# hruffieux/atlasqtl

Measured on AMD Instinct MI355X. Metric: VB sweeps/sec, higher is better.
Workload: dtype f64; 1 GPU; atlasqtl VB sweep (S1-S22 incl. scheduled ELBO), n=1000 p=50000 q=10000, anneal=(1,2,10) on, horseshoe global-local, sweeps 6-93; n=1000, p=50000, q=10000, q_per_gpu=10000, parallelism=trait-sharded x1, env_overrides=

## Files before the change

### atlasqtl_amd/csrc/aq_core_sweep.h

```cpp
#pragma once
#include <hip/hip_runtime.h>
#include "aq_special.h"
#include "aq_plan_const.h"

typedef double aq_d4 __attribute__((ext_vector_type(4)));

struct AqCoreArgs {
  const double2 *XA;
  const double2 *XU;
  const double *G;
  const double *Gx;
  double *R;
  double *gam;
  double *mu;
  const double *Aarr;
  const double *Barr;
  const double *coef;
  const double *inv2s;
  const double *cst;
  const double *sig2b;
  double *sums;
  double *rowGB;
  double c;
  int p, q;
  int p_pad, q_pad, n_pad, nb, ntile;
  int dmode;
  int mode;
  int nseg;
  int stagger;
  int *done;
  int *errflag;
  int C;
  int xtouch;
  int xhelper;
  double *Pbuf;
  int *pflag;
  double *rnpart;
  const double *mis;
  const double *GK;
  const double *tau, *log_tau;
  const double *sig2_inv_p, *log_sig2_inv_p;
  long long *dbg;
  const double *theta;
  const double *zeta;
  double sqrt_c;
  int c_is_one;
  int mprio;
  int hprio;
};

__device__ __forceinline__ aq_d4 aq_mfma(double a, double b, aq_d4 c) {
  return __builtin_amdgcn_mfma_f64_16x16x4f64(a, b, c, 0, 0, 0);
}
__device__ __forceinline__ void aq_lds_barrier() { asm volatile("s_waitcnt lgkmcnt(0)\n\ts_barrier" ::: "memory"); }
__device__ __forceinline__ int aq_drow(int dmode, int reg, int g) { return (dmode ? 1 : 4) * reg + (dmode ? 4 : 1) * g; }
```

### atlasqtl_amd/csrc/aq_core_sweep_la.h

```cpp
#pragma once
#include <hip/hip_runtime.h>
#include "aq_core_sweep.h"
#include <type_traits>

typedef double aq_v2 __attribute__((ext_vector_type(2)));

__device__ __forceinline__ double aq_row16_sum(double v) {
  auto step = [&](auto ctrl) __attribute__((always_inline)) {
    constexpr int C = decltype(ctrl)::value;
    const int lo = __builtin_amdgcn_update_dpp(0, __double2loint(v), C, 0xf, 0xf, false);
    const int hi = __builtin_amdgcn_update_dpp(0, __double2hiint(v), C, 0xf, 0xf, false);
    v += __hiloint2double(hi, lo);
  };
  step(std::integral_constant<int, 0xB1>{});
  step(std::integral_constant<int, 0x4E>{});
  step(std::integral_constant<int, 0x124>{});
  step(std::integral_constant<int, 0x128>{});
  return v;
}

#ifndef AQ_GLDS_AUX
#define AQ_GLDS_AUX 2
#endif
__device__ __forceinline__ void aq_glds16(const void *gsrc_lane, void *lds_base) {
// ... 724 lines not shown
          double gxn[CXC ? RPG : 1];
          if constexpr (CXC) {
#pragma unroll
            for (int r = 0; r < RPG; r++) gxn[r] = LGx[(b + 1) % 3][(hg + NG * r) * 16 + j];
          }
          __builtin_amdgcn_sched_barrier(0);
          double s = sb + m1o * dj;
          double mu = rc_coef * s;
          double x = fma(-(s * s), rc_K, cA);
          double gm = aq_sigmoid_neg_fast(x);
          double dl = gm * mu - m1o;
          sb = s_nx - g_next * dl;
          if (j2 < 16) {
            Sown[j2 / NG] -= gl[j2 / NG] * dl;
            s_nx = __shfl(Sown[j2 / NG], (j2 % NG) * NTR + ht, 64);
            __builtin_amdgcn_sched_barrier(0);
          }
#pragma unroll
          for (int r = (j / NG); r < RPG; r++)
            if (!(j2 < 16 && r == j2 / NG)) Sown[r] -= gl[r] * dl;
          if constexpr (CXC) {
#pragma unroll
            for (int r = 0; r < RPG; r++) cxn[r] = (j == 0 ? 0.0 : cxn[r]) + gxn[r] * dl;
          }
          wgam[j * NTR] = gm;
          wmu[j * NTR] = mu;
          wdel[j * NTR] = dl;
          m1o = m1o_n; cA = cA_n; dj = d_n;
          if (j == 7) tl_mark(need, 6);
        }
        }
        signal(6, b - seg_b0 + 1);
      };
      if constexpr (NT3 > 0) {
        run(std::integral_constant<int, (NT3 > 0 ? NT3 : 1)>{}, std::integral_constant<int, 2>{},
            [&](int i) __attribute__((always_inline)) { if (i >= 1 && i <= nblk) chain_block(seg_b0 + i - 1); });
      } else {
        for (int b = seg_b0; b < seg_b1; b++) chain_block(b);
      }
    } else if constexpr (NT3 > 0) {
      run(std::integral_constant<int, (NT3 > 0 ? NT3 : 1)>{}, std::integral_constant<int, 2>{}, no_hook);
    }
    __syncthreads();
  } else if (helper) {
    if (a.hprio == 3) __builtin_amdgcn_s_setprio(3);
    else if (a.hprio == 2) __builtin_amdgcn_s_setprio(2);
    else if (a.hprio == 1) __builtin_amdgcn_s_setprio(1);
    const size_t tbase = (size_t)(tile0 + (ht >> 4)) * a.p_pad * 16 + (ht & 15);
    const double zk = a.zeta[ktrait];
    typedef __attribute__((address_space(3))) const double aq_lds_cdouble;
    aq_lds_cdouble *ptab = (aq_lds_cdouble *)(__attribute__((address_space(3))) double *)Lpt;
    const double inv_sqrt_c = 1.0 / a.sqrt_c;
    const double cst_k = MASK ? 0.0 : a.cst[ktrait];
    double th[RPG];
    auto theta_load = [&](int b) __attribute__((always_inline)) {
#pragma unroll
      for (int r = 0; r < RPG; r++) th[r] = a.theta[16 * b + hg + NG * r];
    };
    double pg[MASK ? 1 : RPG], pm[MASK ? 1 : RPG];
    auto gm_load = [&](int b) __attribute__((always_inline)) {
      if constexpr (!MASK) {
#pragma unroll
        for (int r = 0; r < RPG; r++) {
          const size_t off = tbase + (size_t)(16 * b + hg + NG * r) * 16;
          pg[r] = a.gam[off];
          pm[r] = a.mu[off];
        }
      }
    };
    const double tau_k = MASK ? a.tau[ktrait] : 1.0;
    const double sig2_inv_h = MASK ? *a.sig2_inv_p : 0.0;
    const double cstna_k = MASK ? -(a.log_tau[ktrait] + *a.log_sig2_inv_p) / 2 : 0.0;
    auto gk_block = [&](int b) __attribute__((always_inline)) { return a.GK + ((size_t)tile0 * a.nb + b) * AQ_GK_STRIDE; };
    auto gk_dma = [&](int b, int par) __attribute__((always_inline)) {
      const char *src = (const char *)gk_block(b) + lane * 16;
#pragma unroll
      for (int i = 0; i < AQ_GK_DIAG / 128; i++) aq_glds16(src + 1024 * i, &LGk2[par][128 * i]);
      src += AQ_GK_DIAG * 8;
#pragma unroll
      for (int i = 0; i < 32; i++) aq_glds16(src + 1024 * i, &LGxk[128 * i]);
    };
    double pl_g[MASK ? RPG : 1], pl_m[MASK ? RPG : 1], pl_xn[MASK ? RPG : 1];
    double sv_g[MASK ? RPG : 1], sv_m[MASK ? RPG : 1], sv_xn[MASK ? RPG : 1], sv_th[MASK ? RPG : 1];
    auto pre_load = [&](int b) __attribute__((always_inline)) {
      const double *gk = gk_block(b);
#pragma unroll
      for (int r = 0; r < RPG; r++) {
        const size_t off = tbase + (size_t)(16 * b + hg + NG * r) * 16;
        const int jj = hg + NG * r;
        pl_g[r] = a.gam[off];
        pl_m[r] = a.mu[off];
        pl_xn[r] = gk[(jj * (jj + 1) / 2 + jj) * 16 + ht];
      }
    };
    auto stage_dma = [&](int b, int par, int b_next) __attribute__((always_inline)) {
#pragma unroll
      for (int r = 0; r < RPG; r++) {
        asm volatile("" : "+v"(pl_g[r]), "+v"(pl_m[r]), "+v"(pl_xn[r]), "+v"(th[r]) : : "memory");
        sv_g[r] = pl_g[r]; sv_m[r] = pl_m[r]; sv_xn[r] = pl_xn[r]; sv_th[r] = th[r];
      }
      gk_dma(b, par);
      if (b_next < seg_b1) { pre_load(b_next); theta_load(b_next); }
    };
    auto stage = [&](int b, int par) __attribute__((always_inline)) {
      double st_G[4], st_Gx[4], st_xn[MASK ? RPG : 1];
      if constexpr (MASK) {
#pragma unroll
        for (int r = 0; r < RPG; r++) { Lm1[par][lane + 64 * r] = sv_g[r] * sv_m[r]; st_xn[r] = sv_xn[r]; }
      } else {
#pragma unroll
        for (int r = 0; r < RPG; r++) Lm1[par][lane + 64 * r] = pg[r] * pm[r];
#pragma unroll
        for (int r = 0; r < 4; r++) {
          st_G[r] = a.G[(size_t)b * 256 + lane + 64 * r];
          const int bx = CXC ? (b + 1 < a.nb ? b + 1 : b) : b;
          st_Gx[r] = a.Gx[(size_t)bx * 256 + lane + 64 * r];
        }
      }
      double ls2r[MASK ? RPG : 1];
      if constexpr (MASK) {
#pragma unroll
        for (int r = 0; r < RPG; r++) {
          const int e = lane + 64 * r;
          const double is2 = a.c * (st_xn[r] + sig2_inv_h) * tau_k;
          const double s2 = aq_recip_pos(is2);
          const double ls2 = -aq_log_pos(is2);
          const double cf = a.c * s2 * tau_k;
          Lcoef[par][e] = cf;
          LK[par][e] = cf * cf * (a.c * 0.5 * is2);
          Ls2[par][e] = s2;
          Lls2[par][e] = ls2;
          Lxn[par][e] = st_xn[r];
          ls2r[r] = ls2;
        }
      }
      auto emitA = [&](int r, double A) __attribute__((always_inline)) {
        const int j = 16 * b + hg + NG * r, e = lane + 64 * r;
        const bool valid = kvalid && j < a.p;
        if constexpr (MASK) {
          LA[par][e] = a.c * ((valid ? A : 0.0) - 0.5 * ls2r[r] + cstna_k);
        } else {
          LA[par][e] = a.c * ((valid ? A : 0.0) + cst_k);
        }
      };
      auto emitZ = [&](int r, double zb, double za) __attribute__((always_inline)) {
        const int j = 16 * b + hg + NG * r, e = lane + 64 * r;
        const bool valid = kvalid && j < a.p;
        LB[par][e] = valid ? zb : 0.0;
        Laa[par][e] = valid ? za : 0.0;
      };
      auto emit2 = [&](int r, double A, double zb, double za) __attribute__((always_inline)) {
        const int j = 16 * b + hg + NG * r, e = lane + 64 * r;
        const bool valid = kvalid && j < a.p;
        LB[par][e] = valid ? zb : 0.0;
        Laa[par][e] = valid ? za : 0.0;
        if constexpr (MASK) LA[par][e] = a.c * ((valid ? A : 0.0) - 0.5 * Lls2[par][e] + cstna_k);
        else LA[par][e] = a.c * ((valid ? A : 0.0) + cst_k);
      };
      double uu[RPG];
      bool inr = true;
#pragma unroll
      for (int r = 0; r < RPG; r++) {
        uu[r] = (MASK ? sv_th[r] : th[r]) + zk;
        inr = inr && fabs(uu[r]) < AQ_PT_R && fabs(a.sqrt_c * uu[r]) < AQ_PT_R;
      }
      {
        constexpr int NC = AQ_PT_DEG + 1, S = AQ_PT_NI, F = NC * S;
        auto locate = [&](double x, double *xloc) __attribute__((always_inline)) {
          const double t = fmin(fabs(x) * (1.0 / AQ_PT_W), AQ_PT_NI * (1.0 - 0x1p-53));
          const int i = (int)t;
          *xloc = fma(2.0, t - (double)i, -1.0);
          return ptab + i;
        };
        {
          double co[2][NC], xl[2];
          auto fetch = [&](int r, auto setc) __attribute__((always_inline)) {
            constexpr int set = decltype(setc)::value;
            aq_lds_cdouble *pp = locate(uu[r], &xl[set]);
#pragma unroll
            for (int k = 0; k < NC; k++) co[set][k] = pp[k * S];
          };
          fetch(0, std::integral_constant<int, 0>{});
          aq_static_for<RPG>([&](auto rc) __attribute__((always_inline)) {
            constexpr int r = decltype(rc)::value, set = r & 1;
            if constexpr (r + 1 < RPG) fetch(r + 1, std::integral_constant<int, (r + 1) & 1>{});
            __builtin_amdgcn_sched_barrier(0);
            double pa = co[set][NC - 1];
#pragma unroll
            for (int k = NC - 2; k >= 0; k--) pa = fma(pa, xl[set], co[set][k]);
            emitA(r, uu[r] < 0.0 ? -pa : pa);
            __builtin_amdgcn_sched_barrier(0);
          });
        }
        {
          double co[2][2 * NC], xl[2];
          auto fetch = [&](int r, auto setc) __attribute__((always_inline)) {
            constexpr int set = decltype(setc)::value;
            aq_lds_cdouble *pp = locate(a.sqrt_c * uu[r], &xl[set]);
#pragma unroll
            for (int k = 0; k < NC; k++) {
              co[set][k] = pp[F + k * S];
              co[set][NC + k] = pp[2 * F + k * S];
            }
          };
          fetch(0, std::integral_constant<int, 0>{});
          aq_static_for<RPG>([&](auto rc) __attribute__((always_inline)) {
            constexpr int r = decltype(rc)::value, set = r & 1;
            if constexpr (r + 1 < RPG) fetch(r + 1, std::integral_constant<int, (r + 1) & 1>{});
            __builtin_amdgcn_sched_barrier(0);
            double pb = co[set][NC - 1], pd = co[set][2 * NC - 1];
#pragma unroll
            for (int k = NC - 2; k >= 0; k--) {
              pb = fma(pb, xl[set], co[set][k]);
              pd = fma(pd, xl[set], co[set][NC + k]);
            }
            const double d = uu[r] < 0.0 ? -pd : pd;
            emitZ(r, pb * inv_sqrt_c, uu[r] - 0.5 * inv_sqrt_c * (pb + d));
            __builtin_amdgcn_sched_barrier(0);
          });
        }
      }
      if (__builtin_expect(!__all(inr), 0)) {
#pragma unroll 1
        for (int r = 0; r < RPG; r++) {
          double ur = uu[0];
#pragma unroll
          for (int k = 1; k < RPG; k++) ur = (r == k) ? uu[k] : ur;
          double A, bM, dM, dummy;
          aq_probit_tab_eval<1>(ur, ptab, &A, &dummy, &dummy);
          aq_probit_tab_eval<2>(a.sqrt_c * ur, ptab, &dummy, &bM, &dM);
          emit2(r, A, bM * inv_sqrt_c, ur - 0.5 * inv_sqrt_c * (bM + dM));
        }
      }
      if constexpr (MASK) {
#ifdef AQ_DIAG_TIME
        const long long t_dma = __builtin_readcyclecounter();
#endif
        asm volatile("s_waitcnt vmcnt(0)" ::: "memory");
#ifdef AQ_DIAG_TIME
        dg_wait += __builtin_readcyclecounter() - t_dma;
#endif
      } else {
#pragma unroll
        for (int r = 0; r < 4; r++) {
          const int e = lane + 64 * r;
          LG[par][(e >> 4) * 32 + (e & 15)] = st_G[r];
          LGx[CXC ? (b + 1) % 3 : par][e] = st_Gx[r];
        }
      }
    };
    double cs0 = 0.0, cs1 = 0.0, cs2 = 0.0, cs3 = 0.0, cs5 = 0.0;
    auto finalize = [&](int b, int par) __attribute__((always_inline)) {
#pragma unroll
      for (int r = 0; r < RPG; r++) {
        const int e = lane + 64 * r, hj = hg + NG * r;
        const double gm = Lgam[par][e], mu = Lmu[par][e];
        const size_t off = tbase + (size_t)(16 * b + hj) * 16;
        if (lead) {
          a.gam[off] = gm;
          a.mu[off] = mu;
        }
        const int j = 16 * b + hj;
        double gb = 0.0;
        if (kvalid && j < a.p) {
          const double be = gm * mu;
          gb = Laa[par][e] + gm * LB[par][e];
          cs0 += gm;
          cs3 += gb;
          if constexpr (MASK) {
            const double s2 = Ls2[par][e];
            const double m2 = (mu * mu + s2) * gm;
            const double xn = Lxn[par][e];
            cs1 += m2;
            cs2 += xn * (m2 - be * be);
            cs5 += gm * Lls2[par][e];
          } else {
            cs1 += (mu * mu + sig2b_k) * gm;
            cs2 += be * be;
          }
        }
        gb = aq_row16_sum(gb);
        if ((ht & 15) == 0 && lead) a.rowGB[(size_t)(tile0 + (ht >> 4)) * a.p_pad + j] = gb;
      }
    };
    auto exchange = [&](int b) __attribute__((always_inline)) {
      const int par = b & 1, kdone = b - seg_b0 + 1;
      if constexpr (WIDE) tl_mark(kdone, 0);
#pragma unroll
      for (int m = 0; m < NWM; m++) wait_ge(m, kdone);
      if constexpr (NT3 > 0) wait_ge(11, kdone);
      if constexpr (WIDE) tl_mark(kdone, 1);
      double own[RPG];
#pragma unroll
      for (int r = 0; r < RPG; r++) {
        const int e = lane + 64 * r;
        double sv = Sp[par][0][e];
#pragma unroll
        for (int ww = 1; ww < NPS; ww++) sv += Sp[par][ww][e];
        own[r] = sv;
      }
      if constexpr (WIDE) split_exchange_wide(b, own, [] {});
      else split_exchange(b, own, [] {});
#pragma unroll
      for (int r = 0; r < RPG; r++) Stot[par][lane + 64 * r] = own[r];
      signal(14, kdone);
    };
    if (a.mode == 1) {
      for (int b = seg_b0; b < seg_b1; b++) {
        const int k = b - seg_b0, par = b & 1;
        if (k >= 2) {
#pragma unroll
          for (int m = 0; m < NWM; m++) wait_ge(m, k + 1);
          if (NT3 > 0) wait_ge(11, k + 1);
        }
#pragma unroll
        for (int r = 0; r < RPG; r++) {
          const int e = lane + 64 * r, hj = hg + NG * r;
          const size_t off = tbase + (size_t)(16 * b + hj) * 16;
          double gm = a.gam[off], mu = a.mu[off];
          double be = gm * mu;
          Ldel[par][e] = be;
          if (kvalid && (16 * b + hj) < a.p) {
            const double m2 = (mu * mu + sig2b_k) * gm;
            cs0 += gm;
            cs1 += m2;
            if constexpr (MASK) cs2 += gk_block(b)[(hj * (hj + 1) / 2 + hj) * 16 + ht] * (m2 - be * be);
            else cs2 += be * be;
          }
        }
        signal(6, k + 1);
      }
    } else {
      int xt[8] = {0, 0, 0, 0, 0, 0, 0, 0};
      const long long xt_blk = (long long)NTT * C * 2048;
      const int xt_nsl = (int)((xt_blk + 8191) / 8192);
      const int xt_wg = (int)(gridDim.x < 256 ? gridDim.x : 256) / 8 > 0 ? (int)(gridDim.x < 256 ? gridDim.x : 256) / 8 : 1;
      auto x_touch = [&](int bA, int bU) __attribute__((always_inline)) {
        asm volatile("s_waitcnt vmcnt(0)" : "+v"(xt[0]), "+v"(xt[1]), "+v"(xt[2]), "+v"(xt[3]), "+v"(xt[4]), "+v"(xt[5]), "+v"(xt[6]), "+v"(xt[7]));
        const char *pa = (const char *)a.XA + (long long)bA * xt_blk + lane * 128, *pu = (const char *)a.XU + (long long)bU * xt_blk + lane * 128;
#pragma unroll
        for (int k = 0; k < 4; k++) {
          const int sl = (int)((blockIdx.x >> 3) % xt_wg) + k * xt_wg;
          if (sl < xt_nsl && (long long)sl * 8192 + lane * 128 < xt_blk) {
            asm volatile("global_load_dword %0, %1, off" : "=v"(xt[2 * k]) : "v"(pa + (long long)sl * 8192));
            asm volatile("global_load_dword %0, %1, off" : "=v"(xt[2 * k + 1]) : "v"(pu + (long long)sl * 8192));
          }
        }
      };
      theta_load(seg_b0);
      gm_load(seg_b0);
      if constexpr (MASK) { pre_load(seg_b0); stage_dma(seg_b0, seg_b0 & 1, seg_b0 + 1); }
      stage(seg_b0, seg_b0 & 1);
      signal(7, 1);
      if constexpr (!SEG && TT == 1) { if (C > 1 && a.xhelper) exchange(seg_b0); }
      if constexpr (!MASK) { if (seg_b0 + 1 < seg_b1) { theta_load(seg_b0 + 1); gm_load(seg_b0 + 1); } }
      for (int b = seg_b0; b < seg_b1; b++) {
        const int par = b & 1;
        if constexpr (MASK) {
          if (b + 1 < seg_b1) { wait_ge(13, b - seg_b0 + 1); stage_dma(b + 1, par ^ 1, b + 2); }
        }
        if (b > seg_b0) {
          wait_ge(6, b - seg_b0);
          if constexpr (!MASK && !CXC) {
            double dlp[16];
#pragma unroll
            for (int i = 0; i < 16; i++) dlp[i] = Ldel[par ^ 1][i * NTR + ht];
#pragma unroll
            for (int r = 0; r < RPG; r++) {
              double cx = 0.0;
              const double *gx = &LGx[par][(hg + NG * r) * 16];
#pragma unroll
              for (int i = 0; i < 16; i++) cx += gx[i] * dlp[i];
              Lcx[lane + 64 * r] = cx;
            }
            signal(12, b - seg_b0 + 1);
          }
          finalize(b - 1, par ^ 1);
        }
        if (b + 1 < seg_b1) {
          stage(b + 1, par ^ 1);
          signal(7, b - seg_b0 + 2);
          if constexpr (!SEG && TT == 1) { if (C > 1 && a.xhelper) exchange(b + 1); }
          if (a.xtouch && b + 2 < seg_b1) x_touch(b + 2, b);
          if constexpr (!MASK) { if (b + 2 < seg_b1) { theta_load(b + 2); gm_load(b + 2); } }
        }
      }
      asm volatile("s_waitcnt vmcnt(0)" : "+v"(xt[0]), "+v"(xt[1]), "+v"(xt[2]), "+v"(xt[3]), "+v"(xt[4]), "+v"(xt[5]), "+v"(xt[6]), "+v"(xt[7]));
      wait_ge(6, nblk);
      finalize(seg_b1 - 1, (seg_b1 - 1) & 1);
    }
    Lred[0][lane] = cs0; Lred[1][lane] = cs1; Lred[2][lane] = cs2; Lred[3][lane] = cs3; Lred[5][lane] = cs5;
    __syncthreads();
  } else {
    if (mw < 3) run(std::integral_constant<int, NT>{}, std::integral_constant<int, 0>{}, no_hook);
    else run(std::integral_constant<int, NT2>{}, std::integral_constant<int, 1>{}, no_hook);
    __syncthreads();
  }
#ifdef AQ_DIAG_TIME
  if (lane == 0 && a.dbg) {
    a.dbg[((size_t)blockIdx.x * 8 + w) * 3] = dg_wait;
    a.dbg[((size_t)blockIdx.x * 8 + w) * 3 + 1] = dg_wait_b;
    a.dbg[((size_t)blockIdx.x * 8 + w) * 3 + 2] = __builtin_readcyclecounter() - dg_t0;
  }
#endif
  if (tid < NTR) {
    int k2 = tile0 * 16 + tid;
    double r2 = 0.0;
    for (int s = 0; s < NPS * 4; s++) r2 += Lrn[s][tid];
    double *sm = a.sums + (size_t)seg * (MASK ? 6 : 5) * a.q_pad;
    if (C > 1) a.rnpart[(size_t)part * a.q_pad + k2] = r2;
    else sm[(size_t)4 * a.q_pad + k2] = r2;
    for (int v = 0; v < 6 && lead; v++) {
      if (v == 4 || (v == 5 && !MASK)) continue;
      double acc2 = 0.0;
      for (int jj = 0; jj < NG; jj++) acc2 += Lred[v][jj * NTR + tid];
      sm[(size_t)v * a.q_pad + k2] = acc2;
    }
  }
  if (SEG) {
    asm volatile("s_waitcnt vmcnt(0)" ::: "memory");
    __syncthreads();
    if (tid == 0) {
      __builtin_amdgcn_fence(__ATOMIC_RELEASE, "agent");
      asm volatile("s_waitcnt vmcnt(0)" ::: "memory");
      __hip_atomic_store(&a.done[wg], seg + 1, __ATOMIC_RELAXED, __HIP_MEMORY_SCOPE_AGENT);
    }
  }
}
```

### atlasqtl_amd/csrc/aq_plan.h

```cpp
#pragma once
#include <algorithm>
#include <cstdio>
#include <cstdlib>
#include <functional>
#include <string>

#include "../../include/atlasqtl_hip.h"
#include "aq_plan_const.h"

struct AqPlanInput {
  int n = 0, p = 0, q = 0;
  bool has_missing = false;
  int max_missing = 0;
  int max_short_list = 0;
  int ncu = 256;
  long long total_bytes = -1;
  const char *mem_error = nullptr;
};

struct AqPlan {
  bool use_la = false;
  bool use_mis = false;
  bool use_tw = false;
  bool la_mask = false;
  bool la_wide = false;
  int NT = 0;
  int NT2 = 0;
  int NT3x = -1;
  int TT = 1;
  int laC = 1;
  int misC = 1;
  int chain = 0;
  int stagger = 0;
  int la_xhelper = 0;
  int la_xtouch = 1;
  int la_hprio = 0;
  int la_mprio = 1;
  int NE = 0;
  int WPT = 1;
  int tw_ns = 4;
  int Mmax = 0, NR = 0;
  int p_pad = 0, q_pad = 0, n_pad = 0, nb = 0, ntile = 0;
  int ncu = 256;
};

using AqEnv = std::function<const char *(const char *)>;

enum AqHook { AQ_H_NCU, AQ_H_KERNEL, AQ_H_LA_C, AQ_H_GK_MAX_GB, AQ_H_MIS_C, AQ_H_TW_WPT, AQ_H_TT, AQ_H_NT3, AQ_H_LA_NOSPLIT,
              AQ_H_LA_XHELPER, AQ_H_XTOUCH, AQ_H_MPRIO, AQ_H_HPRIO, AQ_H_STAGGER, AQ_H_CHAIN, AQ_H_COUNT };
static const char *const aq_hook_names[AQ_H_COUNT] = {"AQ_NCU", "AQ_KERNEL", "AQ_LA_C", "AQ_GK_MAX_GB", "AQ_MIS_C", "AQ_TW_WPT", "AQ_TT", "AQ_NT3",
                                                      "AQ_LA_NOSPLIT", "AQ_LA_XHELPER", "AQ_XTOUCH", "AQ_MPRIO", "AQ_HPRIO", "AQ_STAGGER", "AQ_CHAIN"};
struct AqOpt { bool set = false, seen = false; int v = 0; double d = 0.0; };
struct AqHooks {
  const AqEnv &env;
  AqOpt opt[AQ_H_COUNT];
  const AqOpt &operator[](AqHook h) {
    AqOpt &o = opt[h];
    if (!o.seen) {
      o.seen = true;
      if (const char *v = env ? env(aq_hook_names[h]) : nullptr) { o.set = true; o.v = atoi(v); o.d = atof(v); }
    }
    return o;
  }
};

static inline int aq_plan_fail(std::string *err, int code, const std::string &msg) {
  if (err) *err = msg;
  return code;
}
static inline int aq_round16(int x) { return (x + 15) / 16 * 16; }

static inline int aq_plan_gk_budget(const AqPlanInput &in, AqHooks &h, bool wide, bool *la_mask_ok, std::string *err) {
  const size_t ntile_ = (size_t)(in.q + 15) / 16, nb_ = (size_t)(in.p + 15) / 16;
  const size_t gk_b = ntile_ * nb_ * AQ_GK_STRIDE * sizeof(double);
  const size_t rest_b = 2 * ntile_ * nb_ * 256 * sizeof(double) + 3 * (size_t)(in.n + 64) * nb_ * 16 * sizeof(double) * 2 +
                        3 * ntile_ * (size_t)(in.n + 64) * 16 * sizeof(double);
  const bool mem_known = in.total_bytes >= 0;
  if (wide && !mem_known) return aq_plan_fail(err, AQ_ERR_DEVICE, std::string("hipMemGetInfo: ") + (in.mem_error ? in.mem_error : "failed"));
  if (!mem_known || (!wide && (double)(gk_b + rest_b) * 1.05 > 0.9 * (double)in.total_bytes)) *la_mask_ok = false;
  const AqOpt &e = h[AQ_H_GK_MAX_GB];
  if (e.set && (double)gk_b > e.d * 1e9) *la_mask_ok = false;
  if (wide && !*la_mask_ok) {
    char msg[256];
    snprintf(msg, sizeof msg, "Y with missing values at n = %d: the per-trait Gram blocks need %.1f GB of device memory, which does not "
             "fit; shard the traits (fewer traits per device)", in.n, (double)gk_b / 1e9);
    return aq_plan_fail(err, AQ_ERR_UNSUPPORTED, msg);
  }
  return AQ_OK;
}

static inline int aq_plan_kernel(const AqPlanInput &in, AqHooks &h, AqPlan *pl, bool *wide_out, std::string *err) {
  const AqOpt &ek = h[AQ_H_KERNEL];
  const bool n_la_ok = in.n <= 8 * 16 * 105;
  const AqOpt &ecw = h[AQ_H_LA_C];
  const bool wide = in.n > 10240 || (ecw.set && ecw.v >= 9);
  if (wide && ecw.set && (ecw.v > AQ_LA_CMAX || (in.n > 10240 && ecw.v < 9)))
    return aq_plan_fail(err, AQ_ERR_ARG, "AQ_LA_C: the wide sample split takes 9 ... " + std::to_string(AQ_LA_CMAX) + " parts");
  if (wide && ek.set && ek.v >= 2) return aq_plan_fail(err, AQ_ERR_UNSUPPORTED, "AQ_KERNEL: only the look-ahead kernel serves n > 10240");
  bool la_mask_ok = in.has_missing && n_la_ok && in.max_missing <= AQ_MIS_MMAX && !(ek.set && ek.v >= 2);
  if (wide) la_mask_ok = in.has_missing;
  if (la_mask_ok) {
    const int rc = aq_plan_gk_budget(in, h, wide, &la_mask_ok, err);
    if (rc != AQ_OK) return rc;
  }
// ... 125 lines not shown
    if (tiles >= (1 << 30)) continue;
    const double rounds = (double)(((long long)pl->ntile * C + pl->ncu - 1) / pl->ncu);
    const double cost = rounds * std::max(0.213 * (NT + NT2) + 1.0, 4.5 + 0.2 * (C - 2));
    if (cost < best - 1e-9) { best = cost; pl->laC = C; pl->NT = NT; pl->NT2 = NT2; pl->NT3x = N3x; pl->n_pad = 16 * tiles * C; }
  }
  return best;
}

static inline double aq_plan_la_wide(AqPlan *pl, const AqOpt &ec, int ntiles) {
  auto helper_us = [](int C) { return 8.5 + 0.14 * (C - 12); };
  double best = 1e300;
  pl->la_wide = true;
  const int cf = ec.set ? ec.v : 0;
  for (int C = 9; C <= AQ_LA_CMAX && C <= pl->ncu; C++) {
    if (cf >= 9 && C != cf) continue;
    const int NT = ((ntiles + C - 1) / C + 5) / 6;
    if (NT > 18) continue;
    const double rounds = (double)(((long long)pl->ntile * C + pl->ncu - 1) / pl->ncu);
    const double cost = rounds * std::max(0.213 * 2 * NT + 1.0, helper_us(C));
    if (cost < best - 1e-9) { best = cost; pl->laC = C; pl->NT = NT; pl->NT2 = NT; pl->NT3x = -1; pl->n_pad = 16 * 6 * NT * C; }
  }
  return best;
}

static inline int aq_plan_la(const AqPlanInput &in, AqHooks &h, bool wide, AqPlan *pl, std::string *err) {
  const int ntiles = (in.n + 15) / 16;
  const bool split = !(in.n <= 1056 && !h[AQ_H_LA_C].set);
  pl->TT = (4LL * pl->ntile >= 7LL * pl->ncu) ? 2 : 1;
  const AqOpt &ett = h[AQ_H_TT];
  if (ett.set) pl->TT = ett.v == 2 ? 2 : 1;
  if (pl->la_mask) pl->TT = 1;
  if (split) pl->TT = 1;
  if (pl->TT == 2) {
    pl->q_pad = (in.q + 31) / 32 * 32;
    pl->ntile = pl->q_pad / 16;
  }
  const AqOpt &e3 = h[AQ_H_NT3];
  if (!split) {
    const int rc = aq_plan_la_unsplit(h, pl, e3, ntiles, err);
    if (rc != AQ_OK) return rc;
  } else {
    const AqOpt &ec = h[AQ_H_LA_C];
    const double best = wide ? aq_plan_la_wide(pl, ec, ntiles) : aq_plan_la_medium(pl, e3, ec, ntiles);
    if (best >= 1e300) return aq_plan_fail(err, AQ_ERR_UNSUPPORTED, "no look-ahead geometry for this n");
    pl->la_xhelper = wide ? 1 : 0;
  }
  if (h[AQ_H_LA_XHELPER].set) pl->la_xhelper = h[AQ_H_LA_XHELPER].v != 0;
  if (h[AQ_H_XTOUCH].set) pl->la_xtouch = h[AQ_H_XTOUCH].v != 0;
  if (pl->la_mask && pl->laC <= 1) pl->la_hprio = 1;
  if (pl->TT == 2 && pl->NT >= 8 && (pl->NT3x == 9 || (pl->NT3x < 0 && pl->NT2 == pl->NT - 1))) pl->la_hprio = 1;
  if (h[AQ_H_MPRIO].set) pl->la_mprio = h[AQ_H_MPRIO].v != 0;
  const AqOpt &ehp = h[AQ_H_HPRIO];
  if (ehp.set) pl->la_hprio = ehp.v >= 0 && ehp.v <= 3 ? ehp.v : 0;
  if (pl->TT == 2) pl->stagger = (pl->NT + 2) / 3;
  const AqOpt &est = h[AQ_H_STAGGER];
  if (est.set) pl->stagger = est.v >= 0 ? est.v : 0;
  pl->chain = aq_plan_chain(h, false, pl->ntile / pl->TT, pl->nb, pl->ncu, pl->laC > 1);
  if (pl->la_wide) pl->Mmax = pl->la_mask ? aq_round16(in.max_short_list) : 0;
  else if (pl->la_mask) pl->Mmax = aq_round16(in.max_missing);
  if ((pl->la_wide || pl->la_mask) && pl->Mmax < 16) pl->Mmax = 16;
  if (pl->la_mask) pl->NR = pl->n_pad + 8;
  return AQ_OK;
}

static inline int aq_plan_wide_budget(const AqPlanInput &in, const AqPlan &pl, std::string *err) {
  const double xb = 2.0 * (double)pl.nb * (pl.n_pad / 16) * 128 * sizeof(double);
  const double rb = (pl.la_mask ? 2.0 : 1.0) * (double)pl.ntile * pl.n_pad * 16 * sizeof(double);
  const double gb = pl.la_mask ? (double)pl.ntile * pl.nb * AQ_GK_STRIDE * sizeof(double) + (double)pl.nb * (pl.n_pad + 8) * 16 * sizeof(double) +
                                     (double)pl.ntile * 16 * pl.Mmax * sizeof(int)
                               : 0.0;
  if (in.total_bytes < 0) return aq_plan_fail(err, AQ_ERR_DEVICE, "hipMemGetInfo failed");
  if ((xb + rb + gb) * 1.05 > 0.9 * (double)in.total_bytes) {
    char msg[256];
    snprintf(msg, sizeof msg, "n = %d, p = %d, q = %d: the wide sample split needs %.1f GB of device memory, more than the device holds; "
             "shard the traits (fewer traits per device)", in.n, in.p, in.q, (xb + rb + gb) * 1.05 / 1e9);
    return aq_plan_fail(err, AQ_ERR_UNSUPPORTED, msg);
  }
  return AQ_OK;
}

static inline int aq_make_plan(const AqPlanInput &in, const AqEnv &env, AqPlan *out, std::string *err) {
  if (in.n > AQ_N_MAX)
    return aq_plan_fail(err, AQ_ERR_UNSUPPORTED, "n = " + std::to_string(in.n) + " exceeds the largest supported sample count, n <= " +
                                                     std::to_string(AQ_N_MAX) + " (AQ_N_MAX, the wide sample split)");
  AqHooks h{env, {}};
  AqPlan pl;
  pl.p_pad = aq_round16(in.p);
  pl.q_pad = aq_round16(in.q);
  pl.nb = pl.p_pad / 16;
  pl.ntile = pl.q_pad / 16;
  pl.ncu = in.ncu;
  if (h[AQ_H_NCU].set && h[AQ_H_NCU].v > 0) pl.ncu = h[AQ_H_NCU].v;
  bool wide = false;
  int rc = aq_plan_kernel(in, h, &pl, &wide, err);
  if (rc != AQ_OK) return rc;
  if (pl.use_mis) aq_plan_mis(in, h, &pl);
  else if (pl.use_tw) aq_plan_tw(in, h, &pl);
  else rc = aq_plan_la(in, h, wide, &pl, err);
  if (rc == AQ_OK && pl.la_wide) rc = aq_plan_wide_budget(in, pl, err);
  if (rc != AQ_OK) return rc;
  *out = pl;
  return AQ_OK;
}

static inline int aq_core_kernel_id(const AqPlan &pl) { return pl.use_mis ? 3 : pl.use_tw ? 2 : 0; }
static inline void aq_plan_to_status(const AqPlan &pl, aq_vb_status *st) {
// ... 11 lines not shown
```

### atlasqtl_amd/csrc/aq_vb_create.hip

```cpp
#include <hip/hip_runtime.h>

#include <algorithm>
#include <cmath>
#include <cstdlib>
#include <cstring>
#include <memory>
#include <string>
#include <vector>

#include "aq_vb.h"
#include "aq_setup_kernels.h"

static int aq_upload_padded(double *dst, const double *src, size_t n, size_t n_pad) {
  AQ_HIP(hipMemset(dst, 0, n_pad * sizeof(double)));
  AQ_HIP(hipMemcpy(dst, src, n * sizeof(double), hipMemcpyHostToDevice));
  return AQ_OK;
}

static AqEnv aq_env_recorder(std::string *found) {
  return [found](const char *name) {
    const char *v = getenv(name);
    if (v) *found += (found->empty() ? "" : " ") + std::string(name) + "=" + v;
    return v;
  };
}

extern "C" int64_t aq_vb_reduce_len(int32_t p) { return (int64_t)((p + 15) / 16) * 16 + AQ_RED_EXTRA; }

static std::vector<double> aq_ladder(const double anneal[3]) {
  double k_m = 1.0 / anneal[1];
  int m = (int)std::llround(anneal[2]);
  std::vector<double> l(m);
  int type = (int)std::llround(anneal[0]);
  if (type == 1) {
    double delta = std::pow(k_m, 1.0 / (1 - m)) - 1;
    for (int i = 0; i < m; i++) l[i] = std::pow(1 + delta, 1.0 - (double)(m - i));
  } else if (type == 2) {
    double delta = (1 / k_m - 1) / (m - 1);
    for (int i = 0; i < m; i++) l[i] = 1.0 / (1 + delta * ((double)(m - i) - 1));
  } else {
    double delta = (1 - k_m) / (m - 1);
    for (int i = 0; i < m; i++) l[i] = k_m + delta * (double)i;
  }
  return l;
}


static void aq_fill_args(aq_vb *s) {
  AqCoreArgs &a = s->core_args;
  a.XA = s->XA.get(); a.XU = s->XU.get(); a.G = s->G.get(); a.Gx = s->Gx.get(); a.R = s->R.get(); a.gam = s->gam.get(); a.mu = s->mu.get();
  a.theta = s->theta.get(); a.zeta = s->zeta.get();
  a.Aarr = s->Aarr.get(); a.Barr = s->Barr.get(); a.coef = s->coef.get(); a.inv2s = s->inv2s.get(); a.cst = s->cst.get(); a.sig2b = s->sig2b.get();
  a.sums = s->sums.get(); a.rowGB = s->rowGB.get();
  a.p = s->p; a.q = s->q; a.p_pad = s->p_pad; a.q_pad = s->q_pad; a.n_pad = s->n_pad; a.nb = s->nb; a.ntile = s->ntile;
  a.dmode = s->dmode;
  a.done = s->done.get(); a.errflag = s->errflag.get(); a.stagger = s->stagger;
  a.C = s->laC; a.xhelper = s->la_xhelper; a.Pbuf = s->Pbuf.get(); a.pflag = s->pflag.get(); a.rnpart = s->rnpart.get();
  a.xtouch = s->la_xtouch;
  a.hprio = s->la_hprio;
  a.mprio = s->la_mprio;
  a.mis = s->mis.get(); a.GK = s->GK.get(); a.tau = s->tau.get(); a.log_tau = s->log_tau.get();
  a.sig2_inv_p = &s->sc.get()->sig2_inv; a.log_sig2_inv_p = &s->sc.get()->log_sig2_inv;

  AqMisArgs &m = s->mis_args;
  m.XA = s->XA.get(); m.XU = s->XU.get(); m.G = s->G.get(); m.XR = s->XR.get(); m.R = s->R.get(); m.mis = s->mis.get(); m.gam = s->gam.get(); m.mu = s->mu.get();
  m.Aarr = s->Aarr.get(); m.Barr = s->Barr.get(); m.tau = s->tau.get(); m.log_tau = s->log_tau.get(); m.sig2b = s->sig2b.get(); m.sc = s->sc.get();
  m.midx = s->midx.get(); m.mcnt4 = s->mcnt4.get(); m.sums = s->sums.get(); m.rowGB = s->rowGB.get();
  m.p = s->p; m.q = s->q; m.p_pad = s->p_pad; m.q_pad = s->q_pad; m.n_pad = s->n_pad; m.nb = s->nb; m.ntile = s->ntile;
  m.dmode = s->dmode; m.NR = s->NR; m.Mmax = s->Mmax;
  m.C = s->misC; m.Pbuf = s->Pbuf.get(); m.pflag = s->pflag.get(); m.errflag = s->errflag.get(); m.rnpart = s->rnpart.get();
  m.done = s->done.get();

  AqTwArgs &t = s->tw_args;
  t.X = s->Xcm.get(); t.R = s->R.get(); t.mis = s->mis.get(); t.XN = s->XN.get(); t.gam = s->gam.get(); t.mu = s->mu.get(); t.Aarr = s->Aarr.get(); t.Barr = s->Barr.get();
  t.tau = s->tau.get(); t.log_tau = s->log_tau.get(); t.sig2b = s->sig2b.get(); t.sc = s->sc.get(); t.sums = s->sums.get(); t.rowGB = s->rowGB.get();
  t.n = s->n; t.p = s->p; t.q = s->q; t.n_pad = s->n_pad; t.p_pad = s->p_pad; t.q_pad = s->q_pad; t.ntile = s->ntile;
  t.complete = s->has_missing ? 0 : 1;
  t.ns = s->tw_ns;

  AqPrepass &v = s->pre_args;
  v.theta = s->theta.get(); v.zeta = s->zeta.get(); v.gam = s->gam.get(); v.Aarr = s->Aarr.get(); v.Barr = s->Barr.get(); v.rowA = s->rowA.get();
  v.colApart = s->colApart.get(); v.Hpart = s->Hpart.get(); v.p = s->p; v.q = s->q; v.p_pad = s->p_pad; v.q_pad = s->q_pad;
  v.rows_per_chunk = s->rows_per_chunk;
  v.write_AB = s->fused ? 0 : 1;

  AqQvec &qv = s->qv;
  qv.eta_h = s->eta_h.get(); qv.kappa_h = s->kappa_h.get(); qv.n0 = s->n0.get(); qv.nobs = s->nobs.get();
  qv.zeta = s->zeta.get(); qv.tau = s->tau.get(); qv.sig2b = s->sig2b.get(); qv.log_tau = s->log_tau.get(); qv.eta_vb = s->eta_vb.get();
  qv.kappa_vb = s->kappa_vb.get(); qv.coef = s->coef.get(); qv.inv2s = s->inv2s.get(); qv.cst = s->cst.get(); qv.sums = s->sums.get();
  qv.colApart = s->colApart.get(); qv.nchunk = s->fused ? 0 : s->nHchunk;
  qv.q = s->q; qv.q_pad = s->q_pad; qv.n = s->n; qv.nu_h = s->nu; qv.rho_h = s->rho;
  qv.na = s->has_missing ? 1 : 0;

  AqPvec &pv = s->pv;
  pv.theta = s->theta.get(); pv.sig2_theta = s->sig2_theta.get(); pv.L = s->L.get(); pv.lam2_inv = s->lam2_inv.get(); pv.Q = s->Q.get();
  pv.rsZ = s->red; pv.part = s->ppart.get(); pv.p = s->p; pv.p_pad = s->p_pad; pv.shr = s->shr; pv.m0 = s->m0;
  pv.A2_inv = s->A2_inv; pv.df = (double)s->df;
}

extern "C" int aq_vb_create(const aq_vb_problem *pr, aq_vb_handle *out) {
  if (!pr || !out) return aq_fail(AQ_ERR_ARG, "aq_vb_create: NULL argument");
  *out = nullptr;
  if (pr->n < 2 || pr->p < 1 || pr->q < 1) return aq_fail(AQ_ERR_ARG, "aq_vb_create: n >= 2, p >= 1, q >= 1 required");
  if (pr->q_total < pr->q) return aq_fail(AQ_ERR_ARG, "aq_vb_create: q_total < q");
  if (!pr->X || !pr->Y || !pr->eta || !pr->kappa || !pr->n0 || (!pr->init_generate && (!pr->gam_vb || !pr->mu_beta_vb)) || !pr->sig2_beta_vb ||
      !pr->sig2_theta_vb || !pr->tau_vb || !pr->theta_vb || !pr->zeta_vb)
    return aq_fail(AQ_ERR_ARG, "aq_vb_create: NULL data pointer");
  if (!(pr->tol > 0)) return aq_fail(AQ_ERR_ARG, "tol must be positive");
  if (pr->maxit < 1) return aq_fail(AQ_ERR_ARG, "maxit must be natural.");
  if (pr->has_anneal) {
    int type = (int)std::llround(pr->anneal[0]);
    if (type < 1 || type > 3)
// ... 275 lines not shown
```

Before: 29.36 sweeps/s.

## Specialize helper loop for c==1 and all-valid blocks with scalar base addressing

Splits the helper wave's block loop into template-specialized variants. One handles c==1 (annealing finished), reusing the polynomial table lookup and dropping the sqrt_c scaling. Another skips per-row validity checks for interior blocks. Loads and stores of gamma, mu, G, Gx, theta and rowGB now use wave-uniform scalar bases (readfirstlane) with 32-bit lane offsets, and rowGB is written with one selected store instead of a per-row conditional store. This cuts VALU address arithmetic and branching on the helper path, at the cost of code size from three instantiated loop bodies.

```diff
diff --git a/atlasqtl_amd/csrc/aq_core_sweep.h b/atlasqtl_amd/csrc/aq_core_sweep.h
--- a/atlasqtl_amd/csrc/aq_core_sweep.h
+++ b/atlasqtl_amd/csrc/aq_core_sweep.h
@@ -47,6 +47,7 @@
   int c_is_one;
   int mprio;
   int hprio;
+  int hfast;
 };
 
 __device__ __forceinline__ aq_d4 aq_mfma(double a, double b, aq_d4 c) {
diff --git a/atlasqtl_amd/csrc/aq_core_sweep_la.h b/atlasqtl_amd/csrc/aq_core_sweep_la.h
--- a/atlasqtl_amd/csrc/aq_core_sweep_la.h
+++ b/atlasqtl_amd/csrc/aq_core_sweep_la.h
@@ -800,19 +800,33 @@
     aq_lds_cdouble *ptab = (aq_lds_cdouble *)(__attribute__((address_space(3))) double *)Lpt;
     const double inv_sqrt_c = 1.0 / a.sqrt_c;
     const double cst_k = MASK ? 0.0 : a.cst[ktrait];
+    auto ubase = [&](const void *p0, long long byteoff) __attribute__((always_inline)) {
+      const unsigned long long v = (unsigned long long)((const char *)p0 + byteoff);
+      const unsigned lo = __builtin_amdgcn_readfirstlane((unsigned)v), hi = __builtin_amdgcn_readfirstlane((unsigned)(v >> 32));
+      return (const char *)(((unsigned long long)hi << 32) | lo);
+    };
+    const long long tile_b = (long long)tile0 * a.p_pad * 128;
+    const unsigned vo_e = (unsigned)(ht >> 4) * (unsigned)a.p_pad * 128u + (unsigned)(hg * 16 + (ht & 15)) * 8u;
+    const unsigned vo_row = ((unsigned)(ht >> 4) * (unsigned)a.p_pad + (unsigned)(hg + NG * (ht & 15))) * 8u;
     double th[RPG];
     auto theta_load = [&](int b) __attribute__((always_inline)) {
-#pragma unroll
-      for (int r = 0; r < RPG; r++) th[r] = a.theta[16 * b + hg + NG * r];
+      if constexpr (MASK) {
+#pragma unroll
+        for (int r = 0; r < RPG; r++) th[r] = a.theta[16 * b + hg + NG * r];
+      } else {
+        const char *tb = ubase(a.theta, (long long)b * 128);
+#pragma unroll
+        for (int r = 0; r < RPG; r++) th[r] = *(const double *)(tb + (unsigned)(hg * 8) + NG * 8 * r);
+      }
     };
     double pg[MASK ? 1 : RPG], pm[MASK ? 1 : RPG];
     auto gm_load = [&](int b) __attribute__((always_inline)) {
       if constexpr (!MASK) {
+        const char *gb = ubase(a.gam, tile_b + (long long)b * 2048), *mb = ubase(a.mu, tile_b + (long long)b * 2048);
 #pragma unroll
         for (int r = 0; r < RPG; r++) {
-          const size_t off = tbase + (size_t)(16 * b + hg + NG * r) * 16;
-          pg[r] = a.gam[off];
-          pm[r] = a.mu[off];
+          pg[r] = *(const double *)(gb + vo_e + NG * 128 * r);
+          pm[r] = *(const double *)(mb + vo_e + NG * 128 * r);
         }
       }
     };
@@ -850,7 +864,8 @@
       gk_dma(b, par);
       if (b_next < seg_b1) { pre_load(b_next); theta_load(b_next); }
     };
-    auto stage = [&](int b, int par) __attribute__((always_inline)) {
+    auto stage = [&](int b, int par, auto c1c, auto allvc) __attribute__((always_inline)) {
+      constexpr bool C1 = decltype(c1c)::value, ALLV = decltype(allvc)::value;
       double st_G[4], st_Gx[4], st_xn[MASK ? RPG : 1];
       if constexpr (MASK) {
 #pragma unroll
@@ -858,11 +873,12 @@
       } else {
 #pragma unroll
         for (int r = 0; r < RPG; r++) Lm1[par][lane + 64 * r] = pg[r] * pm[r];
+        const int bx = CXC ? (b + 1 < a.nb ? b + 1 : b) : b;
+        const char *Gb = ubase(a.G, (long long)b * 2048), *Gxb = ubase(a.Gx, (long long)bx * 2048);
 #pragma unroll
         for (int r = 0; r < 4; r++) {
-          st_G[r] = a.G[(size_t)b * 256 + lane + 64 * r];
-          const int bx = CXC ? (b + 1 < a.nb ? b + 1 : b) : b;
-          st_Gx[r] = a.Gx[(size_t)bx * 256 + lane + 64 * r];
+          st_G[r] = *(const double *)(Gb + (unsigned)(lane * 8) + 512 * r);
+          st_Gx[r] = *(const double *)(Gxb + (unsigned)(lane * 8) + 512 * r);
         }
       }
       double ls2r[MASK ? RPG : 1];
@@ -884,16 +900,15 @@
       }
       auto emitA = [&](int r, double A) __attribute__((always_inline)) {
         const int j = 16 * b + hg + NG * r, e = lane + 64 * r;
-        const bool valid = kvalid && j < a.p;
-        if constexpr (MASK) {
-          LA[par][e] = a.c * ((valid ? A : 0.0) - 0.5 * ls2r[r] + cstna_k);
-        } else {
-          LA[par][e] = a.c * ((valid ? A : 0.0) + cst_k);
-        }
+        const bool valid = ALLV || (kvalid && j < a.p);
+        const double Av = valid ? A : 0.0;
+        const double t = MASK ? Av - 0.5 * ls2r[r] + cstna_k
+                              : Av + cst_k;
+        LA[par][e] = C1 ? t : a.c * t;
       };
       auto emitZ = [&](int r, double zb, double za) __attribute__((always_inline)) {
         const int j = 16 * b + hg + NG * r, e = lane + 64 * r;
-        const bool valid = kvalid && j < a.p;
+        const bool valid = ALLV || (kvalid && j < a.p);
         LB[par][e] = valid ? zb : 0.0;
         Laa[par][e] = valid ? za : 0.0;
       };
@@ -910,8 +925,11 @@
 #pragma unroll
       for (int r = 0; r < RPG; r++) {
         uu[r] = (MASK ? sv_th[r] : th[r]) + zk;
-        inr = inr && fabs(uu[r]) < AQ_PT_R && fabs(a.sqrt_c * uu[r]) < AQ_PT_R;
-      }
+        if constexpr (C1) inr = inr && fabs(uu[r]) < AQ_PT_R;
+        else inr = inr && fabs(uu[r]) < AQ_PT_R && fabs(a.sqrt_c * uu[r]) < AQ_PT_R;
+      }
+      aq_lds_cdouble *kp[C1 ? RPG : 1];
+      double kx[C1 ? RPG : 1];
       {
         constexpr int NC = AQ_PT_DEG + 1, S = AQ_PT_NI, F = NC * S;
         auto locate = [&](double x, double *xloc) __attribute__((always_inline)) {
@@ -925,6 +943,7 @@
           auto fetch = [&](int r, auto setc) __attribute__((always_inline)) {
             constexpr int set = decltype(setc)::value;
             aq_lds_cdouble *pp = locate(uu[r], &xl[set]);
+            if constexpr (C1) { kp[r] = pp; kx[r] = xl[set]; }
 #pragma unroll
             for (int k = 0; k < NC; k++) co[set][k] = pp[k * S];
           };
@@ -944,7 +963,9 @@
           double co[2][2 * NC], xl[2];
           auto fetch = [&](int r, auto setc) __attribute__((always_inline)) {
             constexpr int set = decltype(setc)::value;
-            aq_lds_cdouble *pp = locate(a.sqrt_c * uu[r], &xl[set]);
+            aq_lds_cdouble *pp;
+            if constexpr (C1) { pp = kp[r]; xl[set] = kx[r]; }
+            else pp = locate(a.sqrt_c * uu[r], &xl[set]);
 #pragma unroll
             for (int k = 0; k < NC; k++) {
               co[set][k] = pp[F + k * S];
@@ -963,7 +984,8 @@
               pd = fma(pd, xl[set], co[set][NC + k]);
             }
             const double d = uu[r] < 0.0 ? -pd : pd;
-            emitZ(r, pb * inv_sqrt_c, uu[r] - 0.5 * inv_sqrt_c * (pb + d));
+            if constexpr (C1) emitZ(r, pb, uu[r] - 0.5 * (pb + d));
+            else emitZ(r, pb * inv_sqrt_c, uu[r] - 0.5 * inv_sqrt_c * (pb + d));
             __builtin_amdgcn_sched_barrier(0);
           });
         }
@@ -998,19 +1020,28 @@
       }
     };
     double cs0 = 0.0, cs1 = 0.0, cs2 = 0.0, cs3 = 0.0, cs5 = 0.0;
-    auto finalize = [&](int b, int par) __attribute__((always_inline)) {
+    auto finalize = [&](int b, int par, auto allvc) __attribute__((always_inline)) {
+      constexpr bool ALLV = decltype(allvc)::value;
+      const char *gsb = nullptr, *msb = nullptr;
+      if constexpr (!MASK) { gsb = ubase(a.gam, tile_b + (long long)b * 2048); msb = ubase(a.mu, tile_b + (long long)b * 2048); }
+      double rsel = 0.0;
 #pragma unroll
       for (int r = 0; r < RPG; r++) {
         const int e = lane + 64 * r, hj = hg + NG * r;
         const double gm = Lgam[par][e], mu = Lmu[par][e];
-        const size_t off = tbase + (size_t)(16 * b + hj) * 16;
         if (lead) {
-          a.gam[off] = gm;
-          a.mu[off] = mu;
+          if constexpr (MASK) {
+            const size_t off = tbase + (size_t)(16 * b + hj) * 16;
+            a.gam[off] = gm;
+            a.mu[off] = mu;
+          } else {
+            *(double *)(gsb + vo_e + NG * 128 * r) = gm;
+            *(double *)(msb + vo_e + NG * 128 * r) = mu;
+          }
         }
         const int j = 16 * b + hj;
         double gb = 0.0;
-        if (kvalid && j < a.p) {
+        if (ALLV || (kvalid && j < a.p)) {
           const double be = gm * mu;
           gb = Laa[par][e] + gm * LB[par][e];
           cs0 += gm;
@@ -1028,7 +1059,14 @@
           }
         }
         gb = aq_row16_sum(gb);
-        if ((ht & 15) == 0 && lead) a.rowGB[(size_t)(tile0 + (ht >> 4)) * a.p_pad + j] = gb;
+        if constexpr (MASK) {
+          if ((ht & 15) == 0 && lead) a.rowGB[(size_t)(tile0 + (ht >> 4)) * a.p_pad + j] = gb;
+        } else {
+          rsel = (ht & 15) == r ? gb : rsel;
+        }
+      }
+      if constexpr (!MASK) {
+        if ((ht & 15) < RPG && lead) *(double *)(ubase(a.rowGB, ((long long)tile0 * a.p_pad + 16 * b) * 8) + vo_row) = rsel;
       }
     };
     auto exchange = [&](int b) __attribute__((always_inline)) {
@@ -1079,63 +1117,79 @@
         signal(6, k + 1);
       }
     } else {
-      int xt[8] = {0, 0, 0, 0, 0, 0, 0, 0};
       const long long xt_blk = (long long)NTT * C * 2048;
       const int xt_nsl = (int)((xt_blk + 8191) / 8192);
       const int xt_wg = (int)(gridDim.x < 256 ? gridDim.x : 256) / 8 > 0 ? (int)(gridDim.x < 256 ? gridDim.x : 256) / 8 : 1;
-      auto x_touch = [&](int bA, int bU) __attribute__((always_inline)) {
-        asm volatile("s_waitcnt vmcnt(0)" : "+v"(xt[0]), "+v"(xt[1]), "+v"(xt[2]), "+v"(xt[3]), "+v"(xt[4]), "+v"(xt[5]), "+v"(xt[6]), "+v"(xt[7]));
-        const char *pa = (const char *)a.XA + (long long)bA * xt_blk + lane * 128, *pu = (const char *)a.XU + (long long)bU * xt_blk + lane * 128;
-#pragma unroll
-        for (int k = 0; k < 4; k++) {
-          const int sl = (int)((blockIdx.x >> 3) % xt_wg) + k * xt_wg;
-          if (sl < xt_nsl && (long long)sl * 8192 + lane * 128 < xt_blk) {
-            asm volatile("global_load_dword %0, %1, off" : "=v"(xt[2 * k]) : "v"(pa + (long long)sl * 8192));
-            asm volatile("global_load_dword %0, %1, off" : "=v"(xt[2 * k + 1]) : "v"(pu + (long long)sl * 8192));
-          }
-        }
-      };
+      using aq_no = std::false_type;
+      using aq_yes = std::true_type;
       theta_load(seg_b0);
       gm_load(seg_b0);
       if constexpr (MASK) { pre_load(seg_b0); stage_dma(seg_b0, seg_b0 & 1, seg_b0 + 1); }
-      stage(seg_b0, seg_b0 & 1);
+      stage(seg_b0, seg_b0 & 1, aq_no{}, aq_no{});
       signal(7, 1);
       if constexpr (!SEG && TT == 1) { if (C > 1 && a.xhelper) exchange(seg_b0); }
       if constexpr (!MASK) { if (seg_b0 + 1 < seg_b1) { theta_load(seg_b0 + 1); gm_load(seg_b0 + 1); } }
-      for (int b = seg_b0; b < seg_b1; b++) {
-        const int par = b & 1;
-        if constexpr (MASK) {
-          if (b + 1 < seg_b1) { wait_ge(13, b - seg_b0 + 1); stage_dma(b + 1, par ^ 1, b + 2); }
-        }
-        if (b > seg_b0) {
-          wait_ge(6, b - seg_b0);
-          if constexpr (!MASK && !CXC) {
-            double dlp[16];
-#pragma unroll
-            for (int i = 0; i < 16; i++) dlp[i] = Ldel[par ^ 1][i * NTR + ht];
-#pragma unroll
-            for (int r = 0; r < RPG; r++) {
-              double cx = 0.0;
-              const double *gx = &LGx[par][(hg + NG * r) * 16];
-#pragma unroll
-              for (int i = 0; i < 16; i++) cx += gx[i] * dlp[i];
-              Lcx[lane + 64 * r] = cx;
+      int xt[8];
+#pragma unroll
+      for (int k = 0; k < 8; k++) asm volatile("" : "=v"(xt[k]));
+      auto hloop = [&](int &b, int end, auto c1c, auto allvc) __attribute__((always_inline)) {
+        auto x_touch = [&](int bA, int bU) __attribute__((always_inline)) {
+          asm volatile("s_waitcnt vmcnt(0)" : "+v"(xt[0]), "+v"(xt[1]), "+v"(xt[2]), "+v"(xt[3]), "+v"(xt[4]), "+v"(xt[5]), "+v"(xt[6]), "+v"(xt[7]));
+          const char *pa = (const char *)a.XA + (long long)bA * xt_blk + lane * 128, *pu = (const char *)a.XU + (long long)bU * xt_blk + lane * 128;
+#pragma unroll
+          for (int k = 0; k < 4; k++) {
+            const int sl = (int)((blockIdx.x >> 3) % xt_wg) + k * xt_wg;
+            if (sl < xt_nsl && (long long)sl * 8192 + lane * 128 < xt_blk) {
+              asm volatile("global_load_dword %0, %1, off" : "=v"(xt[2 * k]) : "v"(pa + (long long)sl * 8192));
+              asm volatile("global_load_dword %0, %1, off" : "=v"(xt[2 * k + 1]) : "v"(pu + (long long)sl * 8192));
             }
-            signal(12, b - seg_b0 + 1);
-          }
-          finalize(b - 1, par ^ 1);
-        }
-        if (b + 1 < seg_b1) {
-          stage(b + 1, par ^ 1);
-          signal(7, b - seg_b0 + 2);
-          if constexpr (!SEG && TT == 1) { if (C > 1 && a.xhelper) exchange(b + 1); }
-          if (a.xtouch && b + 2 < seg_b1) x_touch(b + 2, b);
-          if constexpr (!MASK) { if (b + 2 < seg_b1) { theta_load(b + 2); gm_load(b + 2); } }
-        }
-      }
-      asm volatile("s_waitcnt vmcnt(0)" : "+v"(xt[0]), "+v"(xt[1]), "+v"(xt[2]), "+v"(xt[3]), "+v"(xt[4]), "+v"(xt[5]), "+v"(xt[6]), "+v"(xt[7]));
+          }
+        };
+        auto iter = [&](int b_) __attribute__((always_inline)) {
+          const int b = __builtin_amdgcn_readfirstlane(b_);
+          const int par = b & 1;
+          if constexpr (MASK) {
+            if (b + 1 < seg_b1) { wait_ge(13, b - seg_b0 + 1); stage_dma(b + 1, par ^ 1, b + 2); }
+          }
+          if (b > seg_b0) {
+            wait_ge(6, b - seg_b0);
+            if constexpr (!MASK && !CXC) {
+              double dlp[16];
+#pragma unroll
+              for (int i = 0; i < 16; i++) dlp[i] = Ldel[par ^ 1][i * NTR + ht];
+#pragma unroll
+              for (int r = 0; r < RPG; r++) {
+                double cx = 0.0;
+                const double *gx = &LGx[par][(hg + NG * r) * 16];
+#pragma unroll
+                for (int i = 0; i < 16; i++) cx += gx[i] * dlp[i];
+                Lcx[lane + 64 * r] = cx;
+              }
+              signal(12, b - seg_b0 + 1);
+            }
+            finalize(b - 1, par ^ 1, allvc);
+          }
+          if (b + 1 < seg_b1) {
+            stage(b + 1, par ^ 1, c1c, allvc);
+            signal(7, b - seg_b0 + 2);
+            if constexpr (!SEG && TT == 1) { if (C > 1 && a.xhelper) exchange(b + 1); }
+            if (a.xtouch && b + 2 < seg_b1) x_touch(b + 2, b);
+            if constexpr (!MASK) { if (b + 2 < seg_b1) { theta_load(b + 2); gm_load(b + 2); } }
+          }
+        };
+        for (; b < end; b++) iter(b);
+        asm volatile("s_waitcnt vmcnt(0)" : "+v"(xt[0]), "+v"(xt[1]), "+v"(xt[2]), "+v"(xt[3]), "+v"(xt[4]), "+v"(xt[5]), "+v"(xt[6]), "+v"(xt[7]));
+      };
+      int b = seg_b0;
+      if constexpr (!WIDE && !(TT == 1 && NT3 == 9)) {
+        const bool fast = a.hfast && (tile0 + TT) * 16 <= a.q, c1 = a.sqrt_c == 1.0 && a.c == 1.0;
+        const int fast_end = !fast ? seg_b0 : ((a.p & 15) != 0 && seg_b1 == a.nb) ? seg_b1 - 2 : seg_b1;
+        hloop(b, c1 ? fast_end : seg_b0, aq_yes{}, aq_yes{});
+        hloop(b, fast_end, aq_no{}, aq_yes{});
+      }
+      hloop(b, seg_b1, aq_no{}, aq_no{});
       wait_ge(6, nblk);
-      finalize(seg_b1 - 1, (seg_b1 - 1) & 1);
+      finalize(seg_b1 - 1, (seg_b1 - 1) & 1, aq_no{});
     }
     Lred[0][lane] = cs0; Lred[1][lane] = cs1; Lred[2][lane] = cs2; Lred[3][lane] = cs3; Lred[5][lane] = cs5;
     __syncthreads();
diff --git a/atlasqtl_amd/csrc/aq_plan.h b/atlasqtl_amd/csrc/aq_plan.h
--- a/atlasqtl_amd/csrc/aq_plan.h
+++ b/atlasqtl_amd/csrc/aq_plan.h
@@ -35,6 +35,7 @@
   int la_xhelper = 0;
   int la_xtouch = 1;
   int la_hprio = 0;
+  int la_hfast = 1;
   int la_mprio = 1;
   int NE = 0;
   int WPT = 1;
@@ -47,9 +48,9 @@
 using AqEnv = std::function<const char *(const char *)>;
 
 enum AqHook { AQ_H_NCU, AQ_H_KERNEL, AQ_H_LA_C, AQ_H_GK_MAX_GB, AQ_H_MIS_C, AQ_H_TW_WPT, AQ_H_TT, AQ_H_NT3, AQ_H_LA_NOSPLIT,
-              AQ_H_LA_XHELPER, AQ_H_XTOUCH, AQ_H_MPRIO, AQ_H_HPRIO, AQ_H_STAGGER, AQ_H_CHAIN, AQ_H_COUNT };
+              AQ_H_LA_XHELPER, AQ_H_XTOUCH, AQ_H_MPRIO, AQ_H_HPRIO, AQ_H_HFAST, AQ_H_STAGGER, AQ_H_CHAIN, AQ_H_COUNT };
 static const char *const aq_hook_names[AQ_H_COUNT] = {"AQ_NCU", "AQ_KERNEL", "AQ_LA_C", "AQ_GK_MAX_GB", "AQ_MIS_C", "AQ_TW_WPT", "AQ_TT", "AQ_NT3",
-                                                      "AQ_LA_NOSPLIT", "AQ_LA_XHELPER", "AQ_XTOUCH", "AQ_MPRIO", "AQ_HPRIO", "AQ_STAGGER", "AQ_CHAIN"};
+                                                      "AQ_LA_NOSPLIT", "AQ_LA_XHELPER", "AQ_XTOUCH", "AQ_MPRIO", "AQ_HPRIO", "AQ_HFAST", "AQ_STAGGER", "AQ_CHAIN"};
 struct AqOpt { bool set = false, seen = false; int v = 0; double d = 0.0; };
 struct AqHooks {
   const AqEnv &env;
@@ -281,6 +282,7 @@
   if (h[AQ_H_MPRIO].set) pl->la_mprio = h[AQ_H_MPRIO].v != 0;
   const AqOpt &ehp = h[AQ_H_HPRIO];
   if (ehp.set) pl->la_hprio = ehp.v >= 0 && ehp.v <= 3 ? ehp.v : 0;
+  if (h[AQ_H_HFAST].set) pl->la_hfast = h[AQ_H_HFAST].v != 0;
   if (pl->TT == 2) pl->stagger = (pl->NT + 2) / 3;
   const AqOpt &est = h[AQ_H_STAGGER];
   if (est.set) pl->stagger = est.v >= 0 ? est.v : 0;
diff --git a/atlasqtl_amd/csrc/aq_vb_create.hip b/atlasqtl_amd/csrc/aq_vb_create.hip
--- a/atlasqtl_amd/csrc/aq_vb_create.hip
+++ b/atlasqtl_amd/csrc/aq_vb_create.hip
@@ -58,6 +58,7 @@
   a.C = s->laC; a.xhelper = s->la_xhelper; a.Pbuf = s->Pbuf.get(); a.pflag = s->pflag.get(); a.rnpart = s->rnpart.get();
   a.xtouch = s->la_xtouch;
   a.hprio = s->la_hprio;
+  a.hfast = s->la_hfast;
   a.mprio = s->la_mprio;
   a.mis = s->mis.get(); a.GK = s->GK.get(); a.tau = s->tau.get(); a.log_tau = s->log_tau.get();
   a.sig2_inv_p = &s->sc.get()->sig2_inv; a.log_sig2_inv_p = &s->sc.get()->log_sig2_inv;
```

New measurement: 28.40 sweeps/s. 0.967x the previous value.
